# talmolab/flybody

Measured on AMD Instinct MI355X. Metric: env-steps/sec (whole node), fruitfly flight-imitation task, higher is better.
Workload: dtype f32; 1 GPU; flight_imitation (BASELINE configs[3]): 4 substeps @5e-5 s (joint limits, fluid forces, the fly's own contacts) + WBPG + obs/reward/termination/auto-reset; envs_per_gpu=8192, global_batch=8192, parallelism=env-sharded x1, actions=uniform over the raw action spec (canonical U(-1,1)), resident in HBM

## Files before the change

flybody_amd/csrc/convex.hpp:

```cpp
#pragma once

#ifdef CVX_HOST
#include <cmath>
#define CVX_FN static inline
namespace dm {
struct V3 { float x, y, z; };
struct Q4 { float w, x, y, z; };
struct M3 { float m0, m1, m2, m3, m4, m5, m6, m7, m8; };
CVX_FN V3 operator+(V3 a, V3 b) { return {a.x + b.x, a.y + b.y, a.z + b.z}; }
CVX_FN V3 operator-(V3 a, V3 b) { return {a.x - b.x, a.y - b.y, a.z - b.z}; }
CVX_FN V3 operator*(float s, V3 a) { return {s * a.x, s * a.y, s * a.z}; }
CVX_FN V3 cross(V3 a, V3 b) { return {a.y * b.z - a.z * b.y, a.z * b.x - a.x * b.z, a.x * b.y - a.y * b.x}; }
CVX_FN float dot(V3 a, V3 b) { return a.x * b.x + a.y * b.y + a.z * b.z; }
CVX_FN M3 q2m(Q4 q) {
  float w = q.w, x = q.x, y = q.y, z = q.z;
  return {w * w + x * x - y * y - z * z, 2 * (x * y - w * z), 2 * (x * z + w * y), 2 * (x * y + w * z), w * w - x * x + y * y - z * z,
          2 * (y * z - w * x), 2 * (x * z - w * y), 2 * (y * z + w * x), w * w - x * x - y * y + z * z};
}
CVX_FN V3 mv(const M3 &m, V3 v) { return {m.m0 * v.x + m.m1 * v.y + m.m2 * v.z, m.m3 * v.x + m.m4 * v.y + m.m5 * v.z, m.m6 * v.x + m.m7 * v.y + m.m8 * v.z}; }
CVX_FN V3 mtv(const M3 &m, V3 v) { return {m.m0 * v.x + m.m3 * v.y + m.m6 * v.z, m.m1 * v.x + m.m4 * v.y + m.m7 * v.z, m.m2 * v.x + m.m5 * v.y + m.m8 * v.z}; }
CVX_FN float frcp(float x) { return 1.f / x; }
CVX_FN float fsqrt(float x) { return x > 0.f ? std::sqrt(x) : 0.f; }
}
#else
// ... 539 lines not shown
      const V3 n = cs * b1 + sn * b2;
      const float o = fsqrt(dot(n, sym_mv(A, n))) + dot(n, c);
      if (o < obest) { obest = o; nbest = n; }
    }
    const float dprev = r.dist;
    za = side(nbest, pe);
    if (r.dist >= 0.f && r.dist > dprev) return r;
  }
  {
    const M3 Re = q2m(e.q);
    const V3 m = e.s0 <= e.s1 && e.s0 <= e.s2 ? V3{Re.m0, Re.m3, Re.m6} : (e.s1 <= e.s2 ? V3{Re.m1, Re.m4, Re.m7} : V3{Re.m2, Re.m5, Re.m8});
    const V3 em = across(m, b1), es = across(pe, V3{-b1.x, -b1.y, -b1.z});
    const float s0 = za > 0.f ? 1.f : -1.f;
    float sr = s0, fb = rim_f(s0, es);
    V3 eb = es;
#pragma unroll
    for (int k = 0; k < 4; k++) {
      const float s = k < 2 ? 1.f : -1.f;
      const V3 e1 = (k & 1) ? em : V3{-em.x, -em.y, -em.z};
      const float f = rim_f(s, e1);
      if (f < fb) { fb = f; sr = s; eb = e1; }
    }
    rim(sr, eb);
    const V3 nb = r.dist > -1e29f ? r.n : V3{-es.x, -es.y, -es.z};
    rim_dual(nb, 1.f);
    rim_dual(nb, -1.f);
    const V3 mt = dot(m, c) > 0.f ? V3{-m.x, -m.y, -m.z} : m;
    rim_dual(mt, 1.f);
    rim_dual(mt, -1.f);
  }
  return r;
}

struct Contact { float dist; V3 n, pos; float t; };

CVX_FN float overlap(const Geom &a, const Geom &b, V3 u) {
  const V3 s1 = support(a, u), s2 = support(b, V3{-u.x, -u.y, -u.z});
  return dot(u, s1 - s2);
}
CVX_FN float separation_bound(const Geom &a, const Geom &b) {
  V3 a1, a2;
  float l1, l2, x1, x2, best = -1e30f;
  core_segment(a, a1, l1); core_segment(b, a2, l2);
  segment_closest(a.c, a1, l1, b.c, a2, l2, x1, x2);
  V3 u = (b.c + x2 * a2) - (a.c + x1 * a1);
  float ul = fsqrt(dot(u, u));
  if (ul > 1e-12f) best = -overlap(a, b, frcp(ul) * u);
  u = b.c - a.c;
  ul = fsqrt(dot(u, u));
  if (ul > 1e-12f) best = fmaxf(best, -overlap(a, b, frcp(ul) * u));
  return best;
}

CVX_FN Contact capsule_capsule(const Geom &a, const Geom &b) {
  const V3 a1 = zaxis(a.q), a2 = zaxis(b.q);
  const float l1 = a.type == CAPSULE ? a.s1 : 0.f, l2 = b.type == CAPSULE ? b.s1 : 0.f;
  float x1, x2;
  {
    const V3 dif = a.c - b.c;
    const float mb = -dot(a1, a2), u = -dot(a1, dif), v = dot(a2, dif), det = 1.f - mb * mb;
    if (fabsf(det) >= 1e-6f) {
      const float idet = 1.f / det;
      x1 = (u - mb * v) * idet; x2 = (v - mb * u) * idet;
      if (x1 > l1) { x1 = l1; x2 = v - mb * l1; } else if (x1 < -l1) { x1 = -l1; x2 = v + mb * l1; }
      if (x2 > l2) { x2 = l2; x1 = fminf(fmaxf(u - mb * l2, -l1), l1); }
      else if (x2 < -l2) { x2 = -l2; x1 = fminf(fmaxf(u + mb * l2, -l1), l1); }
    } else {
      const float c2 = u, lo = fmaxf(-l1, c2 - l2), hi = fminf(l1, c2 + l2);
      x1 = lo <= hi ? 0.5f * (lo + hi) : (c2 > 0.f ? l1 : -l1);
      x2 = fminf(fmaxf((x1 - c2) * (mb < 0.f ? 1.f : -1.f), -l2), l2);
    }
  }
  const V3 q1 = a.c + x1 * a1, q2 = b.c + x2 * a2, d12 = q2 - q1;
  const float cd = fsqrt(dot(d12, d12));
  Contact out;
  out.t = 0.f;
  out.n = cd >= 1e-15f ? frcp(cd) * d12 : V3{1.f, 0.f, 0.f};
  out.dist = cd - a.s0 - b.s0;
  out.pos = q1 + (a.s0 + 0.5f * out.dist) * out.n;
  return out;
}

CVX_FN Result cyl_cyl(const Geom &g1, const Geom &g2) {
  return distance<6, 4>(g1, g2, V3{0.f, 0.f, 0.f}, false, 0.05f * fminf(g1.s0, g2.s0), 1e30f);
}

#ifndef CVX_PRIM_ITERS
#define CVX_PRIM_ITERS 8
#endif
#ifndef CVX_ELLELL_ITERS
#define CVX_ELLELL_ITERS 8
#endif
#ifndef CVX_ELLCYL_ITERS
#define CVX_ELLCYL_ITERS 8
#endif
template <bool WITH_RARE = true>
CVX_FN Contact collide(const Geom &g1, const Geom &g2, V3 n0 = V3{0.f, 0.f, 0.f}, bool have_n = false, float t0 = 0.f) {
  Contact out;
  out.t = 0.f;
  if (g2.type <= CAPSULE) return capsule_capsule(g1, g2);
  if (g1.type <= CAPSULE) {
    const PResult r = prim_convex<CVX_PRIM_ITERS>(g1, g2, t0, have_n);
    out.dist = r.dist; out.n = r.n; out.pos = r.pos; out.t = r.t;
  } else if (g2.type == ELLIPSOID) {
    const Result r = ell_ell<CVX_ELLELL_ITERS>(g1, g2, n0, have_n);
    out.dist = r.dist; out.n = r.n; out.pos = r.pos;
// ... 15 lines not shown
```

flybody_amd/csrc/dev_model.hpp:

```cpp
#pragma once

#include <cmath>
#include <cstdint>
#include <cstring>
#include <map>
#include <stdexcept>
#include <string>
#include <vector>

#if defined(__HIP_DEVICE_COMPILE__)
#define FFE_GLOBAL __attribute__((address_space(1)))
#define FFE_CONST __attribute__((address_space(4)))
#else
#define FFE_GLOBAL
#define FFE_CONST
#endif

namespace ffe {

constexpr int kWave = 64;
constexpr int kMaxLink = 19;
constexpr int kMaxDof = 42;
constexpr int kMaxM = 422;
constexpr int kMaxAct = 16;
constexpr int kMaxWrap = 8;
constexpr int kMaxObsJ = 32;
constexpr int kMaxFuture = 8;
constexpr int kLanePad = 64;
constexpr int kMaxGeom = 72;
constexpr int kMaxPair = 384;

struct Tensor {
  int dtype = 0;
  std::vector<uint32_t> dims;
  const unsigned char *data = nullptr;
  size_t count = 0;
  double f(size_t i) const { double v; std::memcpy(&v, data + 8 * i, 8); return v; }
  int32_t i(size_t k) const { int32_t v; std::memcpy(&v, data + 4 * k, 4); return v; }
};

class Blob {
 public:
  Blob(const void *p, size_t n) {
    const unsigned char *b = static_cast<const unsigned char *>(p);
    if (n < 12 || std::memcmp(b, "FFMB", 4) != 0) throw std::runtime_error("model blob: bad magic");
    uint32_t ver, cnt;
    std::memcpy(&ver, b + 4, 4);
    std::memcpy(&cnt, b + 8, 4);
    if (ver != 1) throw std::runtime_error("model blob: unsupported version");
    size_t off = 12;
    for (uint32_t k = 0; k < cnt; k++) {
      uint16_t nl;
      if (off + 2 > n) throw std::runtime_error("model blob: truncated");
      std::memcpy(&nl, b + off, 2); off += 2;
      std::string name(reinterpret_cast<const char *>(b + off), nl); off += nl;
      Tensor t;
      t.dtype = b[off]; int ndim = b[off + 1]; off += 2;
      t.count = 1;
      for (int d = 0; d < ndim; d++) { uint32_t v; std::memcpy(&v, b + off, 4); off += 4; t.dims.push_back(v); t.count *= v; }
      off += (8 - off % 8) % 8;
      t.data = b + off;
      off += t.count * (t.dtype == 0 ? 8 : 4);
      if (off > n) throw std::runtime_error("model blob: truncated tensor " + name);
      tensors_[name] = t;
    }
  }
  bool has(const std::string &name) const { return tensors_.count(name) != 0; }
  const Tensor &get(const std::string &name) const {
    auto it = tensors_.find(name);
    if (it == tensors_.end()) throw std::runtime_error("model blob: missing tensor " + name);
    return it->second;
  }

 private:
  std::map<std::string, Tensor> tensors_;
};

struct DevModel {
  int nlink, nv, nq, nu, nM, nrootrec, nobsj, nwing, naction, nsub;
  float h, gx, gy, gz, total_mass;
  const int FFE_GLOBAL *d_link, *d_madr, *d_depth, *d_kind, *d_qadr, *d_limited, *d_act_id, *d_ndesc;
  const unsigned int FFE_GLOBAL *pairtab;
  const unsigned int FFE_GLOBAL *br_seq;
  int nbr_steps, nroot;
  int any_b2;
  const unsigned int FFE_GLOBAL *fsched;
  int fs_branch_rounds, fs_rounds, nbranch;
  const float FFE_GLOBAL *d_axis, *d_arm, *d_damp, *d_stiff, *d_sref, *d_lo, *d_hi, *d_margin, *d_invw, *d_K, *d_B, *d_solimp,
      *d_act_coef, *d_qpos0;
  const int FFE_GLOBAL *l_parent, *l_dofadr, *l_dofnum, *l_sub, *l_reckind, *l_recell;
  const unsigned int FFE_GLOBAL *l_anc;
  const float FFE_GLOBAL *l_pos, *l_quat, *l_ipos, *l_imat, *l_inertia, *l_mass, *l_recpos, *l_recmat, *l_reccoef;
  const float FFE_GLOBAL *rr_pos, *rr_mat, *rr_coef;
  const float FFE_GLOBAL *ell;
  const unsigned char FFE_GLOBAL *m_row, *m_col;
  const unsigned short FFE_GLOBAL *colmadr;
  const int FFE_GLOBAL *a_cl, *a_fl, *a_action, *t_qadr, *t_dof;
  const float FFE_GLOBAL *t_coef;
  const float FFE_GLOBAL *a_gain, *a_b0, *a_b1, *a_b2, *a_clo, *a_chi, *a_flo, *a_fhi;
  const int FFE_GLOBAL *wing_dof, *wing_qadr, *wing_action, *wing_ctrl, *obsj_qadr, *obsj_dof;
  int user_action;
  const float FFE_GLOBAL *qpos0;
  int ncg, ncp;
  float c_margin, c_gap, c_K, c_B, c_solimp[5];
  unsigned long long cg_mmask[2];
  const int FFE_GLOBAL *cg_link, *cg_type;
  const float FFE_GLOBAL *cg_pos, *cg_quat, *cg_size, *cg_brad, *cg_invw;
  const unsigned short FFE_GLOBAL *cp_pair;
  const unsigned long long FFE_GLOBAL *l_dofmask;
};

struct BoxCoef { float c[8]; };

inline BoxCoef box_coefs(const double *box, double rho, double beta) {
  const double kPi = 3.14159265358979323846;
  BoxCoef o;
  double diam = (box[0] + box[1] + box[2]) / 3.0;
  o.c[0] = static_cast<float>(beta > 0 ? kPi * diam * diam * diam * beta : 0.0);
  o.c[1] = static_cast<float>(beta > 0 ? 3.0 * kPi * diam * beta : 0.0);
  o.c[2] = static_cast<float>(0.5 * rho * box[1] * box[2]);
  o.c[3] = static_cast<float>(0.5 * rho * box[0] * box[2]);
  o.c[4] = static_cast<float>(0.5 * rho * box[0] * box[1]);
  o.c[5] = static_cast<float>(rho * box[0] * (std::pow(box[1], 4) + std::pow(box[2], 4)) / 64.0);
  o.c[6] = static_cast<float>(rho * box[1] * (std::pow(box[0], 4) + std::pow(box[2], 4)) / 64.0);
  o.c[7] = static_cast<float>(rho * box[2] * (std::pow(box[0], 4) + std::pow(box[1], 4)) / 64.0);
  return o;
}

inline void quat2mat_d(const double *q, double *m) {
  double w = q[0], x = q[1], y = q[2], z = q[3];
  m[0] = w * w + x * x - y * y - z * z; m[1] = 2 * (x * y - w * z); m[2] = 2 * (x * z + w * y);
  m[3] = 2 * (x * y + w * z); m[4] = w * w - x * x + y * y - z * z; m[5] = 2 * (y * z - w * x);
  m[6] = 2 * (x * z - w * y); m[7] = 2 * (y * z + w * x); m[8] = w * w - x * x - y * y + z * z;
}

class Arena {
 public:
  template <typename T>
  size_t put(const std::vector<T> &v) {
    size_t off = (buf_.size() + 15) & ~size_t(15);
    buf_.resize(off + v.size() * sizeof(T) + 16);
    std::memcpy(buf_.data() + off, v.data(), v.size() * sizeof(T));
    return off;
  }
  const std::vector<unsigned char> &bytes() const { return buf_; }

 private:
  std::vector<unsigned char> buf_;
};

struct HostModel {
  DevModel view{};
  std::vector<unsigned char> arena;
  std::vector<float> action_min, action_max;
  std::vector<double> qpos0;
  int nobs = 0;

  void fixup(DevModel &dst, const unsigned char *base) const {
    dst = view;
    auto fix = [&](auto &p) {
      using P = std::remove_reference_t<decltype(p)>;
      p = (P)((size_t)base + (size_t)p);
    };
    fix(dst.d_link); fix(dst.d_madr); fix(dst.d_depth); fix(dst.d_kind); fix(dst.d_qadr);
    fix(dst.d_limited); fix(dst.d_act_id); fix(dst.d_ndesc); fix(dst.pairtab); fix(dst.br_seq); fix(dst.fsched); fix(dst.d_axis); fix(dst.d_arm); fix(dst.d_damp); fix(dst.d_stiff);
    fix(dst.d_sref); fix(dst.d_lo); fix(dst.d_hi); fix(dst.d_margin); fix(dst.d_invw); fix(dst.d_K); fix(dst.d_B);
    fix(dst.d_solimp); fix(dst.d_act_coef); fix(dst.d_qpos0);
    fix(dst.l_anc); fix(dst.l_parent); fix(dst.l_dofadr); fix(dst.l_dofnum); fix(dst.l_sub); fix(dst.l_reckind); fix(dst.l_recell);
    fix(dst.l_pos); fix(dst.l_quat); fix(dst.l_ipos); fix(dst.l_imat); fix(dst.l_inertia); fix(dst.l_mass);
    fix(dst.l_recpos); fix(dst.l_recmat); fix(dst.l_reccoef);
    fix(dst.rr_pos); fix(dst.rr_mat); fix(dst.rr_coef); fix(dst.ell);
    fix(dst.m_row); fix(dst.m_col); fix(dst.colmadr);
    fix(dst.a_cl); fix(dst.a_fl); fix(dst.a_action); fix(dst.t_qadr); fix(dst.t_dof); fix(dst.t_coef);
    fix(dst.a_gain); fix(dst.a_b0); fix(dst.a_b1); fix(dst.a_b2); fix(dst.a_clo); fix(dst.a_chi); fix(dst.a_flo);
    fix(dst.a_fhi);
    fix(dst.wing_dof); fix(dst.wing_qadr); fix(dst.wing_action); fix(dst.wing_ctrl); fix(dst.obsj_qadr); fix(dst.obsj_dof);
    fix(dst.qpos0);
    fix(dst.cg_link); fix(dst.cg_type); fix(dst.cg_pos); fix(dst.cg_quat); fix(dst.cg_size); fix(dst.cg_brad); fix(dst.cg_invw);
    fix(dst.cp_pair); fix(dst.l_dofmask);
  }
};

template <typename P>
inline void set_off(P &p, size_t off) { p = (P)off; }

inline HostModel build_host_model(const Blob &b) {
  HostModel H;
  DevModel &V = H.view;
  Arena A;
  const Tensor &opt = b.get("opt");
  const double h = opt.f(0), rho = opt.f(1), beta = opt.f(2);
  const Tensor &lparent = b.get("link_parent");
  const int nl = static_cast<int>(lparent.count);
  const Tensor &dofpar = b.get("dof_parentid");
  const int nv = static_cast<int>(dofpar.count);
  const int nq = static_cast<int>(b.get("qpos0").count);
  const int nu = static_cast<int>(b.get("act_trntype").count);
  if (nl > kMaxLink || nv > kMaxDof || nu > kMaxAct) throw std::runtime_error("model exceeds kernel capacities");
  V.nlink = nl; V.nv = nv; V.nq = nq; V.nu = nu;
  V.h = static_cast<float>(h);
  V.gx = static_cast<float>(opt.f(3)); V.gy = static_cast<float>(opt.f(4)); V.gz = static_cast<float>(opt.f(5));

  auto lane_f = [&](int comps) { return std::vector<float>(static_cast<size_t>(comps) * kLanePad, 0.f); };
  auto lane_i = [&](int comps, int fill = 0) { return std::vector<int>(static_cast<size_t>(comps) * kLanePad, fill); };

  const Tensor &body_link = b.get("body_link");
  const Tensor &dof_body = b.get("dof_bodyid");
  const Tensor &dof_jnt = b.get("dof_jntid");
  const Tensor &jnt_type = b.get("jnt_type");
  const Tensor &jnt_qadr = b.get("jnt_qposadr");
  const Tensor &jnt_dadr = b.get("jnt_dofadr");
  const Tensor &jnt_axis = b.get("jnt_axis");
  const Tensor &jnt_pos = b.get("jnt_pos");
  for (size_t k = 0; k < jnt_pos.count; k++)
    if (jnt_pos.f(k) != 0.0) throw std::runtime_error("joint anchors away from the body origin are not supported");
  if (jnt_type.i(0) != 0) throw std::runtime_error("root joint must be free");

  auto d_parent = lane_i(1, -1), d_link = lane_i(1), d_madr = lane_i(1), d_depth = lane_i(1), d_kind = lane_i(1),
       d_qadr = lane_i(1), d_limited = lane_i(1), d_act_id = lane_i(2, -1);
  auto d_axis = lane_f(3), d_arm = lane_f(1), d_damp = lane_f(1), d_stiff = lane_f(1), d_sref = lane_f(1),
       d_lo = lane_f(1), d_hi = lane_f(1), d_margin = lane_f(1), d_invw = lane_f(1), d_K = lane_f(1), d_B = lane_f(1),
       d_solimp = lane_f(5), d_act_coef = lane_f(2), d_qpos0 = lane_f(1);
  std::vector<unsigned char> m_row, m_col;
  int maxdepth = 0;
  for (int d = 0; d < nv; d++) {
    d_parent[d] = dofpar.i(d);
    d_link[d] = body_link.i(dof_body.i(d));
    int j = dof_jnt.i(d), jt = jnt_type.i(j);
    int within = d - jnt_dadr.i(j);
    if (jt == 0) { d_kind[d] = within < 3 ? 0 : 1; d_qadr[d] = within % 3; }
    else if (jt == 3) { d_kind[d] = 2; d_qadr[d] = jnt_qadr.i(j); }
// ... 228 lines not shown
      for (int w = ten_adr.i(id); w < ten_adr.i(id) + ten_num.i(id); w++) {
        int dof = wrap_dof.i(w);
        w_dof.push_back(dof); w_qadr.push_back(jnt_qadr.i(dof_jnt.i(dof))); w_coef.push_back(static_cast<float>(wrap_coef.f(w)));
        add_coupling(dof, u, static_cast<float>(gear * wrap_coef.f(w)));
      }
    } else throw std::runtime_error("body (adhesion) transmissions are not supported yet");
  }
  for (int u = nu; u <= kMaxAct; u++) a_wrap_off[u] = static_cast<int>(w_qadr.size());
  V.any_b2 = 0;
  for (int u = 0; u < nu; u++) if (a_b2[u] != 0.f) V.any_b2 = 1;
  std::vector<int> t_qadr(kMaxWrap * kMaxAct, 0), t_dof(kMaxWrap * kMaxAct, 0);
  std::vector<float> t_coef(kMaxWrap * kMaxAct, 0.f);
  for (int u = 0; u < nu; u++) {
    if (a_trn[u] == 0) { t_qadr[u] = a_qadr[u]; t_dof[u] = a_dof[u]; t_coef[u] = 1.f; }
    else {
      int n = a_wrap_off[u + 1] - a_wrap_off[u];
      if (n > kMaxWrap) throw std::runtime_error("tendon with too many joints");
      for (int w = 0; w < n; w++) {
        t_qadr[w * kMaxAct + u] = w_qadr[a_wrap_off[u] + w]; t_dof[w * kMaxAct + u] = w_dof[a_wrap_off[u] + w];
        t_coef[w * kMaxAct + u] = w_coef[a_wrap_off[u] + w];
      }
    }
  }
  if (w_qadr.empty()) { w_qadr.push_back(0); w_dof.push_back(0); w_coef.push_back(0.f); }

  const Tensor &wing_jnt = b.get("wing_jnt"), &wing_act = b.get("wing_action"), &obs_jnt = b.get("obs_jnt");
  std::vector<int> wing_dof(8, 0), wing_qadr(8, 0), wing_action(8, 0), obsj_qadr(kMaxObsJ, 0), obsj_dof(kMaxObsJ, 0);
  V.nwing = static_cast<int>(wing_jnt.count);
  std::vector<int> wing_ctrl(8, -1);
  for (int k = 0; k < V.nwing; k++) {
    wing_dof[k] = jnt_dadr.i(wing_jnt.i(k)); wing_qadr[k] = jnt_qadr.i(wing_jnt.i(k)); wing_action[k] = wing_act.i(k);
    for (int u = 0; u < nu; u++)
      if (a_action[u] == wing_action[k]) {
        if (wing_ctrl[k] >= 0) throw std::runtime_error("a wing action entry feeds more than one actuator");
        wing_ctrl[k] = u;
      }
  }
  std::vector<unsigned short> colmadr(m_row.size() + 8, 0);
  for (size_t e = 0; e < m_row.size(); e++) colmadr[e] = static_cast<unsigned short>(d_madr[m_col[e]]);
  V.nobsj = static_cast<int>(obs_jnt.count);
  if (V.nobsj > kMaxObsJ) throw std::runtime_error("too many observable joints");
  for (int k = 0; k < V.nobsj; k++) { obsj_qadr[k] = jnt_qadr.i(obs_jnt.i(k)); obsj_dof[k] = jnt_dadr.i(obs_jnt.i(k)); }
  V.user_action = b.get("user_action").count ? b.get("user_action").i(0) : -1;
  V.naction = static_cast<int>(b.get("action_min").count);
  for (int k = 0; k < V.naction; k++) { H.action_min.push_back(static_cast<float>(b.get("action_min").f(k))); H.action_max.push_back(static_cast<float>(b.get("action_max").f(k))); }
  std::vector<float> qpos0(nq);
  for (int k = 0; k < nq; k++) { qpos0[k] = static_cast<float>(b.get("qpos0").f(k)); H.qpos0.push_back(b.get("qpos0").f(k)); }
  const Tensor &site = b.get("site");
  for (int c = 1; c <= 3; c++) if (site.f(c) != 0.0) throw std::runtime_error("sensor site must sit at the root body origin");
  if (site.f(4) != 1.0) throw std::runtime_error("sensor site must share the root body orientation");

  std::vector<int> cg_link(kMaxGeom, 0), cg_type(kMaxGeom, 0);
  std::vector<float> cg_pos(3 * kMaxGeom, 0.f), cg_quat(4 * kMaxGeom, 0.f), cg_size(3 * kMaxGeom, 0.f), cg_brad(kMaxGeom, 0.f), cg_invw(kMaxGeom, 0.f);
  std::vector<unsigned short> cp_pair(kMaxPair, 0xffffu);
  std::vector<unsigned long long> l_dofmask(kMaxLink + 1, 0ull);
  V.ncg = V.ncp = 0; V.cg_mmask[0] = V.cg_mmask[1] = 0ull;
  V.c_margin = V.c_gap = V.c_K = V.c_B = 0.f;
  for (int d = 0; d < nv; d++) {
    const int lk = d_link[d];
    for (int k = 0; k < nl; k++) {
      bool below = false;
      for (int a = k; a >= 0; a = lparent.i(a)) below |= (a == lk);
      if (below) l_dofmask[k] |= 1ull << d;
    }
  }
  if (b.has("cgeom_link")) {
    const Tensor &gl = b.get("cgeom_link"), &gp = b.get("cgeom_pos"), &gq = b.get("cgeom_quat"), &gt = b.get("geom_type"), &gs = b.get("geom_size"),
                 &gm = b.get("geom_margin"), &gg = b.get("geom_gap"), &gsr = b.get("geom_solref"), &gsi = b.get("geom_solimp"), &gcd = b.get("geom_condim"),
                 &gb = b.get("geom_bodyid"), &biw = b.get("body_invweight0"), &c1 = b.get("cand_g1"), &c2 = b.get("cand_g2");
    const int ng = static_cast<int>(gl.count);
    if (ng > kMaxGeom || static_cast<int>(c1.count) > kMaxPair) throw std::runtime_error("collision tables exceed kernel capacities");
    V.ncg = ng;
    for (int g = 0; g < ng; g++) {
      const int ty = gt.i(g);
      if (ty < 2 || ty > 5) throw std::runtime_error("flight model: unexpected geom type");
      if (gcd.i(g) != 1) throw std::runtime_error("flight model: fly geoms are expected to be condim 1");
      cg_link[g] = gl.i(g); cg_type[g] = ty;
      for (int c = 0; c < 3; c++) { cg_pos[c * kMaxGeom + g] = static_cast<float>(gp.f(3 * g + c)); cg_size[c * kMaxGeom + g] = static_cast<float>(gs.f(3 * g + c)); }
      for (int c = 0; c < 4; c++) cg_quat[c * kMaxGeom + g] = static_cast<float>(gq.f(4 * g + c));
      const double s0 = gs.f(3 * g), s1 = gs.f(3 * g + 1), s2 = gs.f(3 * g + 2);
      cg_brad[g] = static_cast<float>(ty == 2 ? s0 : ty == 3 ? s0 + s1 : ty == 5 ? std::sqrt(s0 * s0 + s1 * s1) : std::fmax(s0, std::fmax(s1, s2)));
      cg_invw[g] = static_cast<float>(biw.f(2 * gb.i(g)));
      double tc = gsr.f(2 * g), dr = gsr.f(2 * g + 1), dmax = std::fmin(std::fmax(gsi.f(5 * g + 1), 1e-4), 0.9999), K, B;
      if (tc > 0) { tc = std::fmax(tc, 2 * h); K = 1.0 / std::fmax(1e-15, dmax * dmax * tc * tc * dr * dr); B = 2.0 / std::fmax(1e-15, dmax * tc); }
      else { K = -tc / std::fmax(1e-15, dmax * dmax); B = -dr / std::fmax(1e-15, dmax); }
      if (g == 0) { V.c_K = static_cast<float>(K); V.c_B = static_cast<float>(B); for (int c = 0; c < 5; c++) V.c_solimp[c] = static_cast<float>(gsi.f(5 * g + c)); }
      if (static_cast<float>(K) != V.c_K || static_cast<float>(B) != V.c_B) throw std::runtime_error("flight model: geom solref is expected to be uniform");
      for (int c = 0; c < 5; c++) if (static_cast<float>(gsi.f(5 * g + c)) != V.c_solimp[c]) throw std::runtime_error("flight model: geom solimp is expected to be uniform");
      if (gm.f(g) != 0) {
        if (V.c_margin != 0.f && (V.c_margin != static_cast<float>(gm.f(g)) || V.c_gap != static_cast<float>(gg.f(g)))) throw std::runtime_error("flight model: one margin class expected");
        V.c_margin = static_cast<float>(gm.f(g)); V.c_gap = static_cast<float>(gg.f(g));
        V.cg_mmask[g >> 6] |= 1ull << (g & 63);
      }
    }
    for (size_t k = 0; k < c1.count; k++) {
      int g1 = c1.i(k), g2 = c2.i(k);
      if (gt.i(g1) > gt.i(g2)) std::swap(g1, g2);
      if (gl.i(g1) == gl.i(g2)) continue;
      cp_pair[V.ncp++] = static_cast<unsigned short>(g1 | (g2 << 8));
    }
  }
  set_off(V.d_link, A.put(d_link));
  set_off(V.d_madr, A.put(d_madr)); set_off(V.d_depth, A.put(d_depth));
  set_off(V.d_kind, A.put(d_kind)); set_off(V.d_qadr, A.put(d_qadr));
  set_off(V.d_limited, A.put(d_limited)); set_off(V.d_act_id, A.put(d_act_id));
  set_off(V.d_ndesc, A.put(d_ndesc)); set_off(V.pairtab, A.put(pairtab)); set_off(V.br_seq, A.put(br_seq)); set_off(V.fsched, A.put(fsched));
  set_off(V.d_axis, A.put(d_axis)); set_off(V.d_arm, A.put(d_arm));
  set_off(V.d_damp, A.put(d_damp)); set_off(V.d_stiff, A.put(d_stiff));
  set_off(V.d_sref, A.put(d_sref)); set_off(V.d_lo, A.put(d_lo));
  set_off(V.d_hi, A.put(d_hi)); set_off(V.d_margin, A.put(d_margin));
  set_off(V.d_invw, A.put(d_invw)); set_off(V.d_K, A.put(d_K));
  set_off(V.d_B, A.put(d_B)); set_off(V.d_solimp, A.put(d_solimp));
  set_off(V.d_act_coef, A.put(d_act_coef)); set_off(V.d_qpos0, A.put(d_qpos0));
  set_off(V.l_anc, A.put(l_anc));
  set_off(V.l_parent, A.put(l_parent)); set_off(V.l_dofadr, A.put(l_dofadr));
  set_off(V.l_dofnum, A.put(l_dofnum)); set_off(V.l_sub, A.put(l_sub));
  set_off(V.l_reckind, A.put(l_reckind)); set_off(V.l_recell, A.put(l_recell));
  set_off(V.l_pos, A.put(l_pos)); set_off(V.l_quat, A.put(l_quat));
  set_off(V.l_ipos, A.put(l_ipos)); set_off(V.l_imat, A.put(l_imat));
  set_off(V.l_inertia, A.put(l_inertia)); set_off(V.l_mass, A.put(l_mass));
  set_off(V.l_recpos, A.put(l_recpos)); set_off(V.l_recmat, A.put(l_recmat));
  set_off(V.l_reccoef, A.put(l_reccoef));
  set_off(V.rr_pos, A.put(rr_pos)); set_off(V.rr_mat, A.put(rr_mat));
  set_off(V.rr_coef, A.put(rr_coef)); set_off(V.ell, A.put(ell));
  set_off(V.m_row, A.put(m_row)); set_off(V.m_col, A.put(m_col)); set_off(V.colmadr, A.put(colmadr));
  set_off(V.a_cl, A.put(a_cl));
  set_off(V.a_fl, A.put(a_fl)); set_off(V.a_action, A.put(a_action));
  set_off(V.t_qadr, A.put(t_qadr)); set_off(V.t_dof, A.put(t_dof)); set_off(V.t_coef, A.put(t_coef));
  set_off(V.a_gain, A.put(a_gain)); set_off(V.a_b0, A.put(a_b0));
  set_off(V.a_b1, A.put(a_b1)); set_off(V.a_b2, A.put(a_b2));
  set_off(V.a_clo, A.put(a_clo)); set_off(V.a_chi, A.put(a_chi));
  set_off(V.a_flo, A.put(a_flo)); set_off(V.a_fhi, A.put(a_fhi));
  set_off(V.wing_dof, A.put(wing_dof)); set_off(V.wing_qadr, A.put(wing_qadr));
  set_off(V.wing_action, A.put(wing_action)); set_off(V.wing_ctrl, A.put(wing_ctrl));
  set_off(V.obsj_qadr, A.put(obsj_qadr)); set_off(V.obsj_dof, A.put(obsj_dof));
  set_off(V.qpos0, A.put(qpos0));
  set_off(V.cg_link, A.put(cg_link)); set_off(V.cg_type, A.put(cg_type)); set_off(V.cg_pos, A.put(cg_pos)); set_off(V.cg_quat, A.put(cg_quat));
  set_off(V.cg_size, A.put(cg_size)); set_off(V.cg_brad, A.put(cg_brad)); set_off(V.cg_invw, A.put(cg_invw));
  set_off(V.cp_pair, A.put(cp_pair)); set_off(V.l_dofmask, A.put(l_dofmask));
  H.arena = A.bytes();
  return H;
}

}
```

flybody_amd/csrc/fly_env.hip:

```cpp
#include <hip/hip_runtime.h>

#include <cstdio>
#include <cstring>
#include <memory>
#include <string>
#include <vector>

#include "../../include/flybody_env.h"
#include "ball_env.hpp"
#include "dev_model.hpp"
#include "launch_order.hpp"
#include "dev_math.hpp"
#include "convex.hpp"

#ifndef FFE_WAVES_PER_SIMD
#define FFE_WAVES_PER_SIMD 4
#endif

namespace ffe {

constexpr int kMC = 6;
constexpr int kNSD = 16;

struct alignas(64) EnvState {
// ... 322 lines not shown
#define CSTAMP(k)                                                                                  \
  do {                                                                                             \
    __builtin_amdgcn_s_waitcnt(0);                                                                 \
    unsigned long long cs_t1 = __builtin_amdgcn_s_memtime();                                       \
    if (lane == 0) atomicAdd(&g_stamps[k], cs_t1 - cs_t0);                                         \
    cs_t0 = cs_t1;                                                                                 \
  } while (0)
#define CSTAMP_DECL unsigned long long cs_t0 = __builtin_amdgcn_s_memtime()
#else
#define STAMP(k) do {} while (0)
#define CSTAMP(k) do {} while (0)
#define CSTAMP_DECL do {} while (0)
#endif
__device__ __forceinline__ void set_com(Ctx &c, V3 v) { if (c.lane == 0) { c.T.sens[9] = v.x; c.T.sens[10] = v.y; c.T.sens[11] = v.z; } }
__device__ __forceinline__ V3 get_com(const Ctx &c) { return {c.T.sens[9], c.T.sens[10], c.T.sens[11]}; }
#ifdef FFE_TRACE
#define TRACE_HI(c) (((unsigned)(c).nrare & 0xffu) | (((unsigned)(c).nfac & 0xffu) << 8) | ((min((c).tr_coll, 0xffffu)) << 16))
__device__ unsigned long long g_trace[32768][4];
#define TRACE_BEGIN unsigned long long tr_t0 = __builtin_amdgcn_s_memrealtime(); const int tr_prev = cost[order[blockIdx.x]]
#define TRACE_END(slot, tr_extra, tr_hi)                                                                                              \
  do {                                                                                                                         \
    __builtin_amdgcn_s_waitcnt(0);                                                                                             \
    if (threadIdx.x == 0 && (slot) < 32768) {                                                                                  \
      g_trace[slot][0] = tr_t0; g_trace[slot][1] = __builtin_amdgcn_s_memrealtime();                                               \
      g_trace[slot][2] = (unsigned long long)__builtin_amdgcn_s_getreg((31 << 11) | 4) | ((unsigned long long)tr_hi << 32);                                                 \
      g_trace[slot][3] = (__builtin_amdgcn_s_getreg((31 << 11) | 20) & 0xf) | ((unsigned long long)(tr_extra) << 8);  \
    }                                                                                                                          \
  } while (0)
#else
#define TRACE_BEGIN do {} while (0)
#define TRACE_HI(c) 0
#define TRACE_END(slot, tr_extra, tr_hi) do {} while (0)
#endif
#ifdef FFE_ABLATION
#define DBG(c, f) ((c).flags & (f))
#else
#define DBG(c, f) (0)
#endif
enum { DBG_SKIP_FACTOR = 1 << 16, DBG_SKIP_SOLVE = 1 << 17, DBG_SKIP_STAGE1 = 1 << 18, DBG_SKIP_MENTRIES = 1 << 19, DBG_SKIP_GHOST = 1 << 20, DBG_SKIP_WBPG = 1 << 21, DBG_SKIP_OBS = 1 << 22, DBG_NO_CARRY = 1 << 23, DBG_NO_ORDER = 1 << 24 };

struct CollA { float4 gc[kMaxGeom], gq[kMaxGeom]; float lq[kMaxLink][4]; float sdc[kNSD][5], sdn[kNSD][5]; };
constexpr int kCL2 = 24;
struct CollB { unsigned short cl1[128], cl2[kCL2]; float rec[kMC][12]; float cl2n[kCL2][5]; };
static_assert(sizeof(CollA) <= sizeof(Tile::LD), "collision scratch A");
static_assert(sizeof(CollB) <= sizeof(Tile::lT) + sizeof(Tile::lb) + sizeof(Tile::lc) && offsetof(Tile, lc) == offsetof(Tile, lT) + sizeof(Tile::lT) + sizeof(Tile::lb), "collision scratch B");
__device__ __forceinline__ CollA &coll_a(Tile &T) { return *reinterpret_cast<CollA *>(&T.LD[0]); }
__device__ __forceinline__ CollB &coll_b(Tile &T) { return *reinterpret_cast<CollB *>(&T.lT[0][0]); }

__device__ __forceinline__ cvx::Geom load_geom(const CollA &A, const DevModel FFE_CONST &M, int g) {
  const float4 cc = A.gc[g], qq = A.gq[g];
  return cvx::Geom{dm::V3{cc.x, cc.y, cc.z}, dm::Q4{qq.x, qq.y, qq.z, qq.w}, M.cg_size[g], M.cg_size[kMaxGeom + g], M.cg_size[2 * kMaxGeom + g], M.cg_type[g]};
}

template <bool WITH_RARE>
__device__ __forceinline__ int collide_narrow(Tile &T, const DevModel FFE_CONST &M, const int lane, int n2, int nk, int ovf) {
  CollA &A = coll_a(T);
  CollB &B = coll_b(T);
  const unsigned long long mm0 = M.cg_mmask[0], mm1 = M.cg_mmask[1];
  const float mclass = M.c_margin;
  auto pair_margin = [&](int a, int b) {
    const bool ma = a < 64 ? ((mm0 >> a) & 1ull) : ((mm1 >> (a - 64)) & 1ull), mb = b < 64 ? ((mm0 >> b) & 1ull) : ((mm1 >> (b - 64)) & 1ull);
    return (ma || mb) ? mclass : 0.f;
  };
  bool hit = false;
  float dist = 0.f, margin = 0.f, ctt = 0.f;
  dm::V3 nrm = {1.f, 0.f, 0.f}, cpos = {0.f, 0.f, 0.f};
  int a = 0, b = 0;
  unsigned w = 0u;
  if (lane < n2) {
    w = B.cl2[lane];
    a = w & 255; b = w >> 8;
    margin = pair_margin(a, b);
    const float *kn = B.cl2n[lane];
    const cvx::Contact ct = cvx::collide<WITH_RARE>(load_geom(A, M, a), load_geom(A, M, b), dm::V3{kn[0], kn[1], kn[2]}, kn[3] != 0.f, kn[4]);
    dist = ct.dist; nrm = ct.n; cpos = ct.pos; ctt = ct.t;
    hit = dist < margin - (margin != 0.f ? M.c_gap : 0.f);
  }
  {
    const int ta = M.cg_type[a], tb = M.cg_type[b];
    const int prio = lane < n2 ? (cvx::rare_class(ta, tb) ? 2 : (ta >= cvx::ELLIPSOID ? 1 : 0)) : -1;
    const unsigned long long b2 = __ballot(prio == 2), b1 = __ballot(prio == 1), b0 = __ballot(prio == 0), below = (1ull << lane) - 1ull;
    const int pos = nk + (prio == 2 ? __popcll(b2 & below) : prio == 1 ? __popcll(b2) + __popcll(b1 & below) : __popcll(b2) + __popcll(b1) + __popcll(b0 & below));
    if (prio >= 0 && pos < kNSD) { float *o = A.sdn[pos]; o[0] = nrm.x; o[1] = nrm.y; o[2] = nrm.z; o[3] = __int_as_float((int)w); o[4] = ctt; }
  }
  nk = min(nk + n2, kNSD);
  unsigned long long bal = __ballot(hit);
  if (__popcll(bal) > kMC) {
    ovf = 1;
    int rank = 0;
    for (unsigned long long m = bal; m; m &= m - 1) {
      const int j = __ffsll((long long)m) - 1;
      const float dj = __shfl(dist, j);
      if (dj < dist || (dj == dist && j < lane)) rank++;
    }
    hit = hit && rank < kMC;
    bal = __ballot(hit);
  }
  const int n = __popcll(bal), idx = __popcll(bal & ((1ull << lane) - 1ull));
  if (hit) {
    float *o = B.rec[idx];
    o[0] = nrm.x; o[1] = nrm.y; o[2] = nrm.z; o[3] = cpos.x; o[4] = cpos.y; o[5] = cpos.z; o[6] = dist;
    o[7] = margin - (margin != 0.f ? M.c_gap : 0.f); o[8] = M.cg_invw[a] + M.cg_invw[b];
    o[9] = __int_as_float(M.cg_link[a]); o[10] = __int_as_float(M.cg_link[b]); o[11] = __int_as_float((int)w);
  }
  SYNC();
  return n | (ovf << 8) | (nk << 16);
}


__device__ __noinline__ int flight_collide_a(Tile *Tp, const DevModel FFE_CONST *Mp, const int lane, const int ncache) {
  Tile &T = *Tp;
  const DevModel FFE_CONST &M = *Mp;
  CollA &A = coll_a(T);
  CollB &B = coll_b(T);
  const int ncg = M.ncg;
  CSTAMP_DECL;
  for (int g = lane; g < ncg; g += kWave) {
    const int l = M.cg_link[g];
    const float *lq = A.lq[l];
    const dm::Q4 xq = {lq[0], lq[1], lq[2], lq[3]};
    const dm::V3 gp = dm::V3{T.xpos[l][0], T.xpos[l][1], T.xpos[l][2]} + dm::qrot(xq, dm::V3{M.cg_pos[g], M.cg_pos[kMaxGeom + g], M.cg_pos[2 * kMaxGeom + g]});
    const dm::Q4 gq = dm::qnormalize(dm::qmul(xq, dm::Q4{M.cg_quat[g], M.cg_quat[kMaxGeom + g], M.cg_quat[2 * kMaxGeom + g], M.cg_quat[3 * kMaxGeom + g]}));
    A.gc[g] = make_float4(gp.x, gp.y, gp.z, M.cg_brad[g]);
    A.gq[g] = make_float4(gq.w, gq.x, gq.y, gq.z);
  }
  SYNC();
  const unsigned long long mm0 = M.cg_mmask[0], mm1 = M.cg_mmask[1];
  const float mclass = M.c_margin;
  auto pair_margin = [&](int a, int b) {
    const bool ma = a < 64 ? ((mm0 >> a) & 1ull) : ((mm1 >> (a - 64)) & 1ull), mb = b < 64 ? ((mm0 >> b) & 1ull) : ((mm1 >> (b - 64)) & 1ull);
    return (ma || mb) ? mclass : 0.f;
  };
  int n1 = 0, ovf = 0;
  const int ncp = M.ncp;
  unsigned pw[kMaxPair / kWave];
#pragma unroll
  for (int r = 0; r < kMaxPair / kWave; r++) pw[r] = M.cp_pair[r * kWave + lane];
#pragma unroll
  for (int r = 0; r < kMaxPair / kWave; r++) {
    const int base = r * kWave;
    if (base >= ncp) break;
    const unsigned w = pw[r];
    bool pass = false;
    if (w != 0xffffu) {
      const int a = w & 255, b = w >> 8;
      const float4 ca = A.gc[a], cb = A.gc[b];
      const float dx = cb.x - ca.x, dy = cb.y - ca.y, dz = cb.z - ca.z, reach = ca.w + cb.w + pair_margin(a, b);
      pass = dx * dx + dy * dy + dz * dz <= reach * reach;
    }
    const unsigned long long bal = __ballot(pass);
    const int idx = n1 + __popcll(bal & ((1ull << lane) - 1ull));
    if (pass && idx < 128) B.cl1[idx] = (unsigned short)w;
    n1 += __popcll(bal);
  }
  if (n1 > 128) { n1 = 128; ovf = 1; }
  SYNC();
  CSTAMP(17);
  int n2 = 0, nk = 0;
  bool any_rare = false;
#pragma unroll 1
  for (int base = 0; base < n1; base += kWave) {
    bool pass = false, keep = false, have_kn = false;
    unsigned w = 0u;
    dm::V3 kn = {0.f, 0.f, 0.f};
    float kt = 0.f;
    if (base + lane < n1) {
      w = B.cl1[base + lane];
      const int a = w & 255, b = w >> 8;
      const cvx::Geom ga = load_geom(A, M, a), gb = load_geom(A, M, b);
      const float margin = pair_margin(a, b), incl = margin - (margin != 0.f ? M.c_gap : 0.f);
      pass = cvx::separation_bound(ga, gb) <= incl;
      if (pass) {
        int alt = -1;
        for (int k = 0; k < ncache; k++) {
          const int pk = __float_as_int(A.sdc[k][3]);
          if (pk == (int)w) {
            kn = dm::V3{A.sdc[k][0], A.sdc[k][1], A.sdc[k][2]};
            kt = A.sdc[k][4];
            have_kn = true;
          } else if ((pk & 255) == a && M.cg_type[pk >> 8] == gb.type) alt = k;
        }
        if (!have_kn && alt >= 0 && ga.type == cvx::ELLIPSOID) { kn = dm::V3{A.sdc[alt][0], A.sdc[alt][1], A.sdc[alt][2]}; have_kn = true; }
        if (have_kn) keep = -cvx::overlap(ga, gb, kn) > incl;
        pass = !keep;
      }
    }
    any_rare = any_rare || __ballot(pass && cvx::rare_class(M.cg_type[w & 255], M.cg_type[w >> 8])) != 0ull;
    const unsigned long long bal = __ballot(pass), balk = __ballot(keep);
    const int idx = n2 + __popcll(bal & ((1ull << lane) - 1ull)), idk = nk + __popcll(balk & ((1ull << lane) - 1ull));
    if (pass && idx < kCL2) { B.cl2[idx] = (unsigned short)w; float *o = B.cl2n[idx]; o[0] = kn.x; o[1] = kn.y; o[2] = kn.z; o[3] = have_kn ? 1.f : 0.f; o[4] = kt; }
    if (keep && idk < kNSD) { A.sdn[idk][0] = kn.x; A.sdn[idk][1] = kn.y; A.sdn[idk][2] = kn.z; A.sdn[idk][3] = __int_as_float((int)w); A.sdn[idk][4] = kt; }
    n2 += __popcll(bal);
    nk = min(nk + __popcll(balk), kNSD);
  }
  if (n2 > kCL2) { n2 = kCL2; ovf = 1; }
  SYNC();
  CSTAMP(18);
  if (any_rare) return 0x40000000 | n2 | (nk << 8) | (ovf << 16);
  const int r = collide_narrow<false>(T, M, lane, n2, nk, ovf);
  CSTAMP(19);
  return r;
}

__device__ __noinline__ int flight_collide_b(Tile *Tp, const DevModel FFE_CONST *Mp, const int lane, const int packed) {
  return collide_narrow<true>(*Tp, *Mp, lane, packed & 0xff, (packed >> 8) & 0xff, (packed >> 16) & 1);
}

__device__ __forceinline__ void flight_collide(Ctx &c) {
  const DevModel FFE_CONST &M = model(c);
  Tile &T = c.T;
  c.nct = 0;
  if (M.ncg == 0 || (c.flags & FFE_NO_CONTACT)) return;
  CollA &A = coll_a(T);
  CollB &B = coll_b(T);
  if (c.lane < kNSD) { float *o = A.sdc[c.lane]; o[0] = c.sd_nx; o[1] = c.sd_ny; o[2] = c.sd_nz; o[3] = __int_as_float(c.sd_pid); o[4] = c.sd_t; }
  SYNC();
#ifdef FFE_TRACE
  const unsigned long long tr_c0 = __builtin_amdgcn_s_memrealtime();
#endif
  int r = __builtin_amdgcn_readfirstlane(flight_collide_a(&T, c.Mp, c.lane, c.sd_cnt));
  if (r & 0x40000000) {
    r = __builtin_amdgcn_readfirstlane(flight_collide_b(&T, c.Mp, c.lane, r));
    c.nrare++;
  }
#ifdef FFE_TRACE
  c.tr_coll += (unsigned)(__builtin_amdgcn_s_memrealtime() - tr_c0);
#endif
  c.nct = r & 0xff;
  c.ct_ovf |= (r >> 8) & 0xff;
  c.sd_cnt = r >> 16;
  if (c.lane < kNSD) { const float *o = A.sdn[c.lane]; c.sd_nx = o[0]; c.sd_ny = o[1]; c.sd_nz = o[2]; c.sd_pid = __float_as_int(o[3]); c.sd_t = o[4]; }
  if (c.lane < kMC) {
    const float *o = B.rec[c.lane];
    c.ct_nx = o[0]; c.ct_ny = o[1]; c.ct_nz = o[2]; c.ct_px = o[3]; c.ct_py = o[4]; c.ct_pz = o[5]; c.ct_dist = o[6]; c.ct_incl = o[7]; c.ct_invw = o[8];
    c.ct_l1 = __float_as_int(o[9]); c.ct_l2 = __float_as_int(o[10]); c.ct_pid = __float_as_int(o[11]);
  }
  SYNC();
}

__device__ __forceinline__ void stage1(Ctx &c) {
  const DevModel FFE_CONST &M = model(c);
  Tile &T = c.T;
  const int lane = c.lane;
  const bool is_link = lane < M.nlink, is_dof = lane < M.nv;
  const int l_dofadr = M.l_dofadr[lane], l_dofnum = M.l_dofnum[lane], l_sub = M.l_sub[lane];
  const int d_link = M.d_link[lane], d_kind = M.d_kind[lane];
  const unsigned anc_lo = M.l_anc[lane], anc_hi = M.l_anc[kLanePad + lane];
  STAMP(8);
  const int d_plink_ = M.l_parent[d_link], d_dof0_ = M.l_dofadr[d_link];
  const float l_mass_ = M.l_mass[lane];
  const V3 l_ipos_ = ldv_lane(M.l_ipos, lane), l_inertia_ = ldv_lane(M.l_inertia, lane);
  const M3 l_imat_ = ldm_lane(M.l_imat, lane);

  if (is_link) {
    Q4 q;
    V3 p;
    if (lane == 0) {
      q = qnormalize(Q4{T.qpos[3], T.qpos[4], T.qpos[5], T.qpos[6]});
      p = {0.f, 0.f, 0.f};
    } else {
      Q4 qr = {1.f, 0.f, 0.f, 0.f};
      V3 jax[3];
      int jqa[3];
      float jq0[3];
#pragma unroll
      for (int j = 0; j < 3; j++) {
        const int d = l_dofadr + (j < l_dofnum ? j : 0);
        jax[j] = ldv_lane(M.d_axis, d); jqa[j] = M.d_qadr[d]; jq0[j] = M.d_qpos0[d];
      }
#pragma unroll
      for (int j = 2; j >= 0; j--) {
        if (j < l_dofnum) {
          const int d = l_dofadr + j;
// ... 1473 lines not shown
```

Measured before the change: 10.91 million env-steps/s.

## Use precomputed unified shape table for separation bounds and register-based contact cache lookup

Adds a per-geom unified shape descriptor (semi-axes, half-length, core axis), built on the host and stored as two float4 rows. The separation-bound and overlap tests now use one branch-light support function over this descriptor instead of type-dispatched support code. The separating-direction cache lookup now scans the cached pair ids and type keys held in lane registers with readlane, instead of reading the LDS cache and doing a global type lookup per entry. This is meant to cut divergence and memory traffic in the collision midphase, at the cost of an extra model table and a cache scan that now runs in every lane, including lanes whose pair did not pass.

```diff
diff --git a/flybody_amd/csrc/convex.hpp b/flybody_amd/csrc/convex.hpp
--- a/flybody_amd/csrc/convex.hpp
+++ b/flybody_amd/csrc/convex.hpp
@@ -615,6 +615,51 @@
   return best;
 }
 
+struct UShape { float ex, ey, ez, h, kx, ky, kz, kh; };
+#ifdef CVX_HOST
+static inline
+#else
+__host__ __device__ inline
+#endif
+UShape ushape(int type, float s0, float s1, float s2) {
+  UShape u{s0, s0, s0, 0.f, 0.f, 0.f, 1.f, 0.f};
+  if (type == ELLIPSOID) {
+    const float mx = fmaxf(fmaxf(s0, s1), s2), mid = s0 + s1 + s2 - mx - fminf(fminf(s0, s1), s2);
+    u.ey = s1; u.ez = s2;
+    u.kx = s0 == mx ? 1.f : 0.f; u.ky = s0 != mx && s1 == mx ? 1.f : 0.f; u.kz = s0 != mx && s1 != mx ? 1.f : 0.f;
+    u.kh = mx - mid;
+  } else if (type == CAPSULE) {
+    u.h = u.kh = s1;
+  } else if (type == CYLINDER) {
+    u.ez = 0.f; u.h = u.kh = s1;
+  }
+  return u;
+}
+struct GeomU { V3 c; M3 R; float ex, ey, ez, h; V3 ka; float kh; };
+CVX_FN GeomU make_u(V3 c, Q4 q, const UShape &s) {
+  GeomU g;
+  g.c = c; g.R = q2m(q);
+  g.ex = s.ex; g.ey = s.ey; g.ez = s.ez; g.h = s.h;
+  g.ka = mv(g.R, V3{s.kx, s.ky, s.kz}); g.kh = s.kh;
+  return g;
+}
+CVX_FN float hsupport_u(const GeomU &g, V3 n) {
+  const V3 l = mtv(g.R, n), el = {g.ex * l.x, g.ey * l.y, g.ez * l.z};
+  return fsqrt(dot(el, el)) + g.h * fabsf(l.z);
+}
+CVX_FN float overlap_u(const GeomU &a, const GeomU &b, V3 u) { return hsupport_u(a, u) + hsupport_u(b, u) - dot(u, b.c - a.c); }
+CVX_FN float separation_bound_u(const GeomU &a, const GeomU &b) {
+  float x1, x2, best = -1e30f;
+  segment_closest(a.c, a.ka, a.kh, b.c, b.ka, b.kh, x1, x2);
+  V3 u = (b.c + x2 * b.ka) - (a.c + x1 * a.ka);
+  float ul = fsqrt(dot(u, u));
+  if (ul > 1e-12f) best = -overlap_u(a, b, frcp(ul) * u);
+  u = b.c - a.c;
+  ul = fsqrt(dot(u, u));
+  if (ul > 1e-12f) best = fmaxf(best, -overlap_u(a, b, frcp(ul) * u));
+  return best;
+}
+
 CVX_FN Contact capsule_capsule(const Geom &a, const Geom &b) {
   const V3 a1 = zaxis(a.q), a2 = zaxis(b.q);
   const float l1 = a.type == CAPSULE ? a.s1 : 0.f, l2 = b.type == CAPSULE ? b.s1 : 0.f;
diff --git a/flybody_amd/csrc/dev_model.hpp b/flybody_amd/csrc/dev_model.hpp
--- a/flybody_amd/csrc/dev_model.hpp
+++ b/flybody_amd/csrc/dev_model.hpp
@@ -7,6 +7,8 @@
 #include <stdexcept>
 #include <string>
 #include <vector>
+
+#include "convex.hpp"
 
 #if defined(__HIP_DEVICE_COMPILE__)
 #define FFE_GLOBAL __attribute__((address_space(1)))
@@ -106,6 +108,7 @@
   unsigned long long cg_mmask[2];
   const int FFE_GLOBAL *cg_link, *cg_type;
   const float FFE_GLOBAL *cg_pos, *cg_quat, *cg_size, *cg_brad, *cg_invw;
+  const float4 FFE_GLOBAL *cg_ush;
   const unsigned short FFE_GLOBAL *cp_pair;
   const unsigned long long FFE_GLOBAL *l_dofmask;
 };
@@ -176,7 +179,7 @@
     fix(dst.a_fhi);
     fix(dst.wing_dof); fix(dst.wing_qadr); fix(dst.wing_action); fix(dst.wing_ctrl); fix(dst.obsj_qadr); fix(dst.obsj_dof);
     fix(dst.qpos0);
-    fix(dst.cg_link); fix(dst.cg_type); fix(dst.cg_pos); fix(dst.cg_quat); fix(dst.cg_size); fix(dst.cg_brad); fix(dst.cg_invw);
+    fix(dst.cg_link); fix(dst.cg_type); fix(dst.cg_pos); fix(dst.cg_quat); fix(dst.cg_size); fix(dst.cg_brad); fix(dst.cg_invw); fix(dst.cg_ush);
     fix(dst.cp_pair); fix(dst.l_dofmask);
   }
 };
@@ -511,6 +514,8 @@
 
   std::vector<int> cg_link(kMaxGeom, 0), cg_type(kMaxGeom, 0);
   std::vector<float> cg_pos(3 * kMaxGeom, 0.f), cg_quat(4 * kMaxGeom, 0.f), cg_size(3 * kMaxGeom, 0.f), cg_brad(kMaxGeom, 0.f), cg_invw(kMaxGeom, 0.f);
+  std::vector<cvx::UShape> cg_ush(kMaxGeom, cvx::UShape{});
+  static_assert(sizeof(cvx::UShape) == 2 * sizeof(float4), "cg_ush rows are read as two float4");
   std::vector<unsigned short> cp_pair(kMaxPair, 0xffffu);
   std::vector<unsigned long long> l_dofmask(kMaxLink + 1, 0ull);
   V.ncg = V.ncp = 0; V.cg_mmask[0] = V.cg_mmask[1] = 0ull;
@@ -540,6 +545,7 @@
       const double s0 = gs.f(3 * g), s1 = gs.f(3 * g + 1), s2 = gs.f(3 * g + 2);
       cg_brad[g] = static_cast<float>(ty == 2 ? s0 : ty == 3 ? s0 + s1 : ty == 5 ? std::sqrt(s0 * s0 + s1 * s1) : std::fmax(s0, std::fmax(s1, s2)));
       cg_invw[g] = static_cast<float>(biw.f(2 * gb.i(g)));
+      cg_ush[g] = cvx::ushape(ty, cg_size[g], cg_size[kMaxGeom + g], cg_size[2 * kMaxGeom + g]);
       double tc = gsr.f(2 * g), dr = gsr.f(2 * g + 1), dmax = std::fmin(std::fmax(gsi.f(5 * g + 1), 1e-4), 0.9999), K, B;
       if (tc > 0) { tc = std::fmax(tc, 2 * h); K = 1.0 / std::fmax(1e-15, dmax * dmax * tc * tc * dr * dr); B = 2.0 / std::fmax(1e-15, dmax * tc); }
       else { K = -tc / std::fmax(1e-15, dmax * dmax); B = -dr / std::fmax(1e-15, dmax); }
@@ -595,7 +601,7 @@
   set_off(V.obsj_qadr, A.put(obsj_qadr)); set_off(V.obsj_dof, A.put(obsj_dof));
   set_off(V.qpos0, A.put(qpos0));
   set_off(V.cg_link, A.put(cg_link)); set_off(V.cg_type, A.put(cg_type)); set_off(V.cg_pos, A.put(cg_pos)); set_off(V.cg_quat, A.put(cg_quat));
-  set_off(V.cg_size, A.put(cg_size)); set_off(V.cg_brad, A.put(cg_brad)); set_off(V.cg_invw, A.put(cg_invw));
+  set_off(V.cg_size, A.put(cg_size)); set_off(V.cg_brad, A.put(cg_brad)); set_off(V.cg_invw, A.put(cg_invw)); set_off(V.cg_ush, A.put(cg_ush));
   set_off(V.cp_pair, A.put(cp_pair)); set_off(V.l_dofmask, A.put(l_dofmask));
   H.arena = A.bytes();
   return H;
diff --git a/flybody_amd/csrc/fly_env.hip b/flybody_amd/csrc/fly_env.hip
--- a/flybody_amd/csrc/fly_env.hip
+++ b/flybody_amd/csrc/fly_env.hip
@@ -398,6 +398,11 @@
   return cvx::Geom{dm::V3{cc.x, cc.y, cc.z}, dm::Q4{qq.x, qq.y, qq.z, qq.w}, M.cg_size[g], M.cg_size[kMaxGeom + g], M.cg_size[2 * kMaxGeom + g], M.cg_type[g]};
 }
 
+__device__ __forceinline__ cvx::UShape ush(const DevModel FFE_CONST &M, int g) {
+  const float4 u = M.cg_ush[2 * g], k = M.cg_ush[2 * g + 1];
+  return cvx::UShape{u.x, u.y, u.z, u.w, k.x, k.y, k.z, k.w};
+}
+
 template <bool WITH_RARE>
 __device__ __forceinline__ int collide_narrow(Tile &T, const DevModel FFE_CONST &M, const int lane, int n2, int nk, int ovf) {
   CollA &A = coll_a(T);
@@ -454,7 +459,7 @@
 }
 
 
-__device__ __noinline__ int flight_collide_a(Tile *Tp, const DevModel FFE_CONST *Mp, const int lane, const int ncache) {
+__device__ __noinline__ int flight_collide_a(Tile *Tp, const DevModel FFE_CONST *Mp, const int lane, const int ncache_, const int cpid) {
   Tile &T = *Tp;
   const DevModel FFE_CONST &M = *Mp;
   CollA &A = coll_a(T);
@@ -502,6 +507,9 @@
   if (n1 > 128) { n1 = 128; ovf = 1; }
   SYNC();
   CSTAMP(17);
+  const int ncache = __builtin_amdgcn_readfirstlane(ncache_);
+  int ckey = -1;
+  if (lane < ncache) ckey = (cpid & 255) | (M.cg_type[min((cpid >> 8) & 255, kMaxGeom - 1)] << 8);
   int n2 = 0, nk = 0;
   bool any_rare = false;
 #pragma unroll 1
@@ -513,21 +521,29 @@
     if (base + lane < n1) {
       w = B.cl1[base + lane];
       const int a = w & 255, b = w >> 8;
-      const cvx::Geom ga = load_geom(A, M, a), gb = load_geom(A, M, b);
+      const float4 ca = A.gc[a], qa = A.gq[a], cb = A.gc[b], qb = A.gq[b];
+      const cvx::UShape sa = ush(M, a), sb = ush(M, b);
+      const cvx::GeomU ga = cvx::make_u(dm::V3{ca.x, ca.y, ca.z}, dm::Q4{qa.x, qa.y, qa.z, qa.w}, sa), gb = cvx::make_u(dm::V3{cb.x, cb.y, cb.z}, dm::Q4{qb.x, qb.y, qb.z, qb.w}, sb);
+      const int ta = M.cg_type[a], tb = M.cg_type[b];
       const float margin = pair_margin(a, b), incl = margin - (margin != 0.f ? M.c_gap : 0.f);
-      pass = cvx::separation_bound(ga, gb) <= incl;
+      pass = cvx::separation_bound_u(ga, gb) <= incl;
+      int hit = -1, alt = -1;
+      const int akey = a | (tb << 8);
+#pragma unroll 1
+      for (int k = 0; k < ncache; k++) {
+        const int pk = __builtin_amdgcn_readlane(cpid, k), kk = __builtin_amdgcn_readlane(ckey, k);
+        if (pk == (int)w) hit = k;
+        else if (kk == akey) alt = k;
+      }
       if (pass) {
-        int alt = -1;
-        for (int k = 0; k < ncache; k++) {
-          const int pk = __float_as_int(A.sdc[k][3]);
-          if (pk == (int)w) {
-            kn = dm::V3{A.sdc[k][0], A.sdc[k][1], A.sdc[k][2]};
-            kt = A.sdc[k][4];
-            have_kn = true;
-          } else if ((pk & 255) == a && M.cg_type[pk >> 8] == gb.type) alt = k;
+        const int k = hit >= 0 ? hit : (ta == cvx::ELLIPSOID ? alt : -1);
+        if (k >= 0) {
+          const float *o = A.sdc[k];
+          kn = dm::V3{o[0], o[1], o[2]};
+          kt = hit >= 0 ? o[4] : 0.f;
+          have_kn = true;
+          keep = -cvx::overlap_u(ga, gb, kn) > incl;
         }
-        if (!have_kn && alt >= 0 && ga.type == cvx::ELLIPSOID) { kn = dm::V3{A.sdc[alt][0], A.sdc[alt][1], A.sdc[alt][2]}; have_kn = true; }
-        if (have_kn) keep = -cvx::overlap(ga, gb, kn) > incl;
         pass = !keep;
       }
     }
@@ -564,7 +580,7 @@
 #ifdef FFE_TRACE
   const unsigned long long tr_c0 = __builtin_amdgcn_s_memrealtime();
 #endif
-  int r = __builtin_amdgcn_readfirstlane(flight_collide_a(&T, c.Mp, c.lane, c.sd_cnt));
+  int r = __builtin_amdgcn_readfirstlane(flight_collide_a(&T, c.Mp, c.lane, c.sd_cnt, c.sd_pid));
   if (r & 0x40000000) {
     r = __builtin_amdgcn_readfirstlane(flight_collide_b(&T, c.Mp, c.lane, r));
     c.nrare++;
```

Measured after the change: 11.31 million env-steps/s, median of 6. +3.7%, better.
